# fulcrumgenomics/fgumi

Hardware: AMD Instinct MI355X
Metric: simplex consensus throughput, input raw reads/s (depth-8 x 150bp) (higher is better)
Workload: dtype f64

## Files before the change

### fgumi_amd/csrc/api.cpp

```cpp
#include <chrono>
#include <cstdio>
#include <stdexcept>
#include <cstring>
#include <mutex>
#include <map>
#include <mutex>
#include <string>
#include <thread>
#include "engine.h"
#include <gnu/libc-version.h>
#include <cmath>
#include "fastpath.h"
#include "host_common.h"
#include "simgen.h"
#include "canon_core.h"
#include "reject_core.h"
#include "aln_tags_core.h"

namespace fgx {
using canon::CANON_KIND_DUPLEX; using canon::CANON_KIND_CODEC; using canon::CANON_KIND_SIMPLEX;
uint32_t launch_canon_molecules(hipStream_t s, int kind, const canon::Params& P, const canon::CodecParams& PC, const uint8_t* d_blob,
                                const uint64_t* d_rec_off, const uint32_t* d_rec_len, const uint32_t* d_grp_first, const uint32_t* d_def, uint32_t nd,
                                const uint64_t* d_first, uint8_t* d_out, const uint64_t* d_out_off, uint32_t* d_out_len, int* d_status,
                                canon::Delta* d_delta, DevBuf& slabs, canon::RefRuns* d_runs, const rej::Params* PS);
// ... 1361 lines not shown
  out4[0] = out4[1] = out4[2] = out4[3] = 0;
  if (c && c->fast) { const FastPath& f = c->fast->fp; out4[0] = f.last_packed_families; out4[1] = f.last_classic_families; out4[2] = f.last_split_build; out4[3] = f.last_first_stage_retries; }
}
void fgx_debug_split_first_slice(double mean_records, int packed, uint32_t* out4) {
  if (!out4) return;
  out4[0] = s2_first_slice_bytes(mean_records, packed != 0);
  out4[1] = out4[0] - s2_tile_bytes(mean_records);
  out4[2] = (uint32_t)sizeof(FullItem);
  out4[3] = S2_FLAG_DESC_BYTES;
}
void fgx_debug_last_packed_rows(const fgx_caller* c, uint64_t* out2) {
  if (!out2) return;
  out2[0] = out2[1] = 0;
  if (c && c->fast) { out2[0] = c->fast->fp.last_packed_clean; out2[1] = c->fast->fp.last_packed_general; }
}
void fgx_debug_last_full_results(const fgx_caller* c, uint64_t* out4) {
  if (!out4) return;
  for (int i = 0; i < 4; i++) out4[i] = (c && c->fast) ? c->fast->fp.last_full_results[i] : 0;
}
uint64_t fgx_debug_last_full_results_over(const fgx_caller* c) { return (c && c->fast) ? c->fast->fp.last_full_results[4] : 0; }
int fgx_debug_full_range_whole(uint32_t base, uint32_t items, uint32_t cap) { return full_range_whole(base, items, cap) ? 1 : 0; }
void fgx_debug_last_chain(const fgx_caller* c, uint32_t* out2) { if (out2) { out2[0] = (c && c->fast) ? c->fast->fp.last_launches : 0u; out2[1] = (c && c->fast) ? c->fast->fp.last_host_syncs : 0u; } }
uint32_t fgx_debug_last_routed(const fgx_caller* c) { return (c && c->fast) ? c->fast->fp.last_routed : 0u; }
int fgx_debug_last_direct(const fgx_caller* c) { return (c && c->fast) ? c->fast->fp.last_direct : 0; }
void fgx_set_general_only(fgx_caller* c, int on) { if (c) c->general_only = on != 0; }
void fgx_set_fast_lds_bytes(fgx_caller* c, uint32_t bytes) { if (c) { if (!c->fast) c->fast = new FastState(); c->fast->fp.lds_tile_bytes_large = bytes; } }

int fgx_call_columns(fgx_caller* c, const uint8_t* bases, const uint8_t* quals, uint32_t n_cols, uint32_t depth, uint8_t* out_base,
                     uint8_t* out_qual, uint32_t* out_depth, uint32_t* out_errors) {
  if (!c) return 1;
// ... 143 lines not shown
```

### fgumi_amd/csrc/fastpath.h

```cpp
#pragma once
#include <algorithm>
#include "engine.h"

#if defined(__HIPCC__)
#define FP_HD __host__ __device__ __forceinline__
#else
#define FP_HD inline
#endif

namespace fgx {

constexpr int FAST_RX_CAP = 48;

struct EndDesc {
  uint64_t col_off;
  uint64_t first_off;
  uint64_t kept_off;
  uint32_t cons_len;
  uint32_t rec_size;
  uint16_t mi_off, cb_off;
  uint8_t mi_len, cb_len, rx_len, type;
  uint8_t has_cb, has_rx, valid, meth;
  char rx[FAST_RX_CAP];
};
// ... 41 lines not shown
  return mean_need > floor16 ? std::min<uint32_t>((mean_need + 15u) & ~15u, 17408u) : floor16;
}
constexpr uint32_t FULL_ITEM_OBS = 0x80000000u;
constexpr uint32_t FULL_ITEM_CONT = 0x40000000u;

struct FullResult {
  uint32_t w0;
  uint32_t w1;
};
static_assert(sizeof(FullResult) == 8, "a result is one 8-byte store");
constexpr uint32_t FULL_RESULT_NONE = 0xFFu;
constexpr uint32_t FULL_RESULT_MAX_ITEMS = 64;
#ifndef FGX_FULL_RESULTS_DEFAULT
#define FGX_FULL_RESULTS_DEFAULT 1
#endif
constexpr int FULL_STATS_N = 5, FULL_STATS_STRIDE = 8;
FP_HD uint64_t full_range_word(uint32_t first, uint32_t items, bool whole) {
  return (uint64_t)first | ((uint64_t)(items < 0xFFFFu ? items : 0xFFFFu) << 32) | ((uint64_t)(whole ? 1u : 0u) << 48);
}
FP_HD bool full_range_whole(uint32_t base, uint32_t items, uint32_t cap) { return base < cap && items <= cap - base; }
FP_HD bool emit_pair_takes(uint32_t Lc1, uint32_t Lc2, uint32_t name_len, uint32_t rg_len, uint32_t mi_len, uint32_t cbl1, uint32_t cbl2,
                                                uint32_t rxl1, uint32_t rxl2, bool same_first, uint64_t dcol, uint64_t dout) {
  return Lc1 >= 8u && Lc1 <= 256u && Lc2 >= 8u && Lc2 <= 256u && name_len + 1u <= 32u && rg_len + 4u <= 32u && mi_len + 4u <= 32u &&
         cbl1 + 4u <= 32u && cbl2 + 4u <= 32u && rxl1 + 4u <= 32u && rxl2 + 4u <= 32u && rxl1 <= (uint32_t)FAST_RX_CAP && rxl2 <= (uint32_t)FAST_RX_CAP &&
         same_first && dcol < (1ull << 30) && dout - 1ull < (1ull << 30) - 1ull;
}
FP_HD bool full_results_family(bool packed, bool pair, bool whole, uint32_t items, bool pair_taken) {
  return packed && pair && whole && items <= FULL_RESULT_MAX_ITEMS && pair_taken;
}

struct SplitRec {
// ... 22 lines not shown
  uint16_t qc, sc;
};
struct SplitOut {
  uint8_t status;
  uint8_t ne;
  uint8_t type_a;
  uint8_t fk_a, fk_b;
  uint8_t kept_a, kept_b;
  uint8_t n;
  uint16_t lc_a, lc_b;
  uint32_t rej;
  uint32_t ov_agree, ov_dis, ov_corr;
  uint32_t depth_stats;
};
static_assert(sizeof(SplitRec) == 32 && sizeof(SplitFam) == 32 && sizeof(SplitOut) == 32, "split descriptors are moved as two 16-byte pieces");

struct SlotDesc {
  uint64_t out_off;
  uint32_t lc_seq;
  uint32_t sum_depth;
};
constexpr uint64_t FULL_DEST_DIRECT = 1ull << 62;

struct FastParams {
  const uint8_t* blob; const uint64_t* rec_off; const uint32_t* rec_len; const uint32_t* grp_first;
  uint32_t g0;
  const DeviceTables* T; const DeviceTables* TU;
  uint32_t min_reads; int64_t max_reads;
  char tag0, tag1, cell0, cell1;
  uint32_t min_input_bq, min_cons_bq, trim, overlap, per_base_tags, track_rejects;
// ... 98 lines not shown
  uint32_t last_deep_families = 0;
  DevBuf d_deep_sizes, d_deep_row0, d_deep_rows, d_deep_fams, d_deep_out, d_deep_out2;
  DevBuf d_deep_walk;
  uint32_t last_duplex_deep = 0;
  uint32_t last_duplex_deep_capped = 0;
  bool canon_second_pass = false;
  bool rejects_pass = false;
  uint32_t last_wide_families = 0;
  DevBuf d_wide_scratch, d_wide_pass, d_wide_pass0, d_wide_depth;
  DevBuf d_mflag, d_mu, d_mt, d_mslot, d_mcontigs;
  const void* ref_runs = nullptr;
  uint32_t last_meth_device = 0;
  uint32_t last_meth_clipped = 0;
  uint32_t last_routed = 0;
  uint64_t last_packed_clean = 0, last_packed_general = 0;
  uint64_t last_packed_families = 0, last_classic_families = 0;
  uint32_t last_split_build = 0;
  uint32_t last_first_stage_retries = 0;
  uint32_t last_launches = 0, last_host_syncs = 0;
  DevBuf d_dir_size, d_dir_off, d_dir_base, d_slot_desc, d_slot_err, d_out2, d_scan_tmp2;
  bool direct_off = false;
  uint64_t dir_cap_min = 0;
  uint32_t dir_chunks_run = 0;
  int last_direct = 0;
  uint32_t lds_wave_bytes = 6144;
  uint32_t lds_wave_bytes_duplex = 8704;
  uint32_t lds_wave_bytes_codec = 5120;
  hipEvent_t ev[4] = {nullptr, nullptr, nullptr, nullptr};
  uint32_t pool_slack = 256; bool pool_init = false;
  uint32_t pool_div = 8;
// ... 13 lines not shown
```

### fgumi_amd/csrc/fastpath.hip

```cpp
#if !defined(FGX_WAVEMU)
#include <hipcub/hipcub.hpp>
#endif
#include "bamrec.h"
#include "canon_core.h"
#include "engine.h"
#include <cstdlib>
#include <memory>
#include <string>
#include <type_traits>
#include "fastpath.h"
#include "gate_core.h"
#include "packed_core.h"
#include "record_core.h"

#if defined(FGX_WAVEMU)
#define FGX_DYN_LDS(name) uint8_t* const name = wavemu::dyn_lds()
#define FGX_PIN(...) ((void)0)
#define FGX_UNDEF4(a, b, c, d) do { a = 0; b = 0; c = 0; d = 0; } while (0)
#define FGX_MEM_PIN() ((void)0)
#define FGX_CONST_AS
#else
#define FGX_DYN_LDS(name) extern __shared__ __align__(16) uint8_t name[]
#define FGX_PIN(...) asm volatile("" : __VA_ARGS__)
#define FGX_UNDEF4(a, b, c, d) asm volatile("" : "=v"(a), "=v"(b), "=v"(c), "=v"(d))
// ... 2547 lines not shown
  uint32_t lb = mx > 33 ? (mx - 33) * 2 / 3 + 1 : 1;
  uint32_t ends = (b - a) < max_ends ? (b - a) : max_ends;
  bound[g] = (uint64_t)ends * lb + COL_BOUND_PAD;
  uint64_t lo = 0;
  uint32_t span = 0xFFFFFFFFu;
  if (b > a) {
    lo = rec_off[a];
    const uint64_t hi = rec_off[b - 1] + rec_len[b - 1];
    if (hi >= lo && hi - lo < 0xFFFFFFFFull) span = (uint32_t)(hi - lo);
  }
  fam_desc[g] = make_uint4((uint32_t)lo, (uint32_t)(lo >> 32), span, b - a);
}

__global__ void k_reduce_stats(const unsigned long long* __restrict__ slots, unsigned long long* __restrict__ out, const unsigned long long* __restrict__ full_stats, uint32_t full_out) {
  uint32_t k = threadIdx.x;
  if (k >= 32 && k < 32 + FULL_STATS_N) {
    unsigned long long v = 0;
    for (int i = 0; i < STAT_SLOTS; i++) v += full_stats[(size_t)i * FULL_STATS_STRIDE + (k - 32)];
    out[full_out + (k - 32)] = v;
  }
  if (k >= 32) return;
  unsigned long long v = 0;
  for (int i = 0; i < STAT_SLOTS; i++) v += slots[(size_t)i * 32 + k];
  out[k < FGX_STATS_LEN ? k : 40 + (k - FGX_STATS_LEN)] = v;
}

}

#define FGX_SYNC(st) do { fp.last_host_syncs++; hip_check(hipStreamSynchronize(st), "sync"); } while (0)
#define FGX_LAUNCH(kernel, grid, block, lds, st, ...) do { fp.last_launches++; hipLaunchKernelGGL((kernel), grid, block, lds, st, __VA_ARGS__); hip_check(hipGetLastError(), #kernel " launch"); } while (0)

// ... 16 lines not shown
enum MiscWord : uint32_t {
  MISC_STATS = 0,
  MISC_COLS_USED = 28,
  MISC_N_DEFERRED = 29,
  MISC_N_METH_CLIPPED = 30,
  MISC_N_RETRY = 31,
  MISC_N_RETRY_OLD = 32,
  MISC_N_ROUTE = 33,
  MISC_SMALL_RECS = 35,
  MISC_DIR_FLAGS = 36,
  MISC_N_BIG = 37,
  MISC_N_DEEP = 38,
  MISC_BUILD_FAMILIES = 40,
  MISC_N_SLOW = 44,
  MISC_FULL_RESULTS = 46,
  MISC_READ_BACK = 51,
  MISC_WORDS = 52
};
constexpr uint32_t MISC_SPLIT_WINDOW = MISC_N_BIG - MISC_N_RETRY + 1;
static_assert(FGX_STATS_LEN <= MISC_COLS_USED && MISC_BUILD_FAMILIES == 40 && MISC_BUILD_FAMILIES + (32 - FGX_STATS_LEN) <= MISC_N_SLOW,
              "k_reduce_stats writes words [0, FGX_STATS_LEN) and 40 .. of misc");
static_assert(MISC_N_METH_CLIPPED == MISC_N_DEFERRED + 1 && MISC_N_METH_CLIPPED < MISC_READ_BACK, "meth_clipped_counter: the word behind the deferred count");
static_assert(MISC_N_RETRY < MISC_N_ROUTE && MISC_N_ROUTE < MISC_N_BIG && MISC_SPLIT_WINDOW == 7 && MISC_N_SLOW < MISC_READ_BACK && MISC_READ_BACK <= MISC_WORDS, "misc layout");

inline bool env_not0(const char* e) { return !(e && e[0] == '0'); }
inline bool env_is1(const char* e) { return e && e[0] == '1'; }
inline int env_int(const char* e, int dflt) { return e ? atoi(e) : dflt; }
inline uint32_t env_in(const char* e, int lo, int hi, uint32_t dflt) { const int v = e ? atoi(e) : 0; return v >= lo && v <= hi ? (uint32_t)v : dflt; }

struct ProcessSwitches {
  const bool v2 = env_not0(fgx_knob("FGX_V2")), seg = env_not0(fgx_knob("FGX_SEG"));
  const bool seg2 = env_is1(fgx_knob("FGX_SEG2"));
  const bool early = env_not0(fgx_knob("FGX_S2_EARLY"));
  const int chunks = env_int(getenv("FGX_SPLIT_CHUNKS"), 0);
  const int nosum = env_int(fgx_knob("FGX_S2_NOSUM"), 1);
  const int packed = env_int(getenv("FGX_S2_PACKED"), 1);
  const bool clean_rows = env_not0(getenv("FGX_S2_CLEAN_ROWS"));
  const bool full_results = FGX_FULL_RESULTS_DEFAULT ? env_not0(getenv("FGX_FULL_RESULTS")) : env_is1(getenv("FGX_FULL_RESULTS"));
  const int s2_debug = env_int(fgx_knob("FGX_S2_DEBUG"), 0);
  const int pace = env_int(fgx_knob("FGX_S2_PACE"), 1);
  const uint32_t s2_bytes = env_in(fgx_knob("FGX_S2_BYTES"), 2048, 32768, 0) & ~15u, s2_wpb = env_in(fgx_knob("FGX_S2_WPB"), 1, 4, 0);
  const int s2_partner = env_int(fgx_knob("FGX_S2_PARTNER"), -1);
  const int s2_fixed = env_int(fgx_knob("FGX_S2_FIXED"), -1);
  const bool later_packed = env_not0(fgx_knob("FGX_S2_LATER_PACKED"));
  const bool verbose = env_is1(fgx_knob("FGX_S2_VERBOSE"));
  const uint32_t seg_wpb = env_in(fgx_knob("FGX_SEG_WPB"), 1, WAVES_PER_BLOCK, WAVES_PER_BLOCK), w2_wpb = env_in(fgx_knob("FGX_W2_WPB"), 1, WAVES_PER_BLOCK, FGX_W2_WPB_DEFAULT),
                 fw_wpb = env_in(fgx_knob("FGX_FW_WPB"), 1, WAVES_PER_BLOCK, WAVES_PER_BLOCK);
};
struct BatchSwitches {
  const char* const split_env = getenv("FGX_SPLIT");
  const bool split = env_not0(split_env);
  const int split_mode = env_int(split_env, 1);
// ... 99 lines not shown
    }
    return d.p;
  }
  FastParams stage_params(uint32_t bytes, bool retry) {
    hip_check(hipMemsetAsync(cnt(MISC_N_RETRY), 0, 4, s), "memset");
    FastParams PS = P;
    PS.group_list = cur_list; PS.lds_wave_bytes = bytes;
    PS.retry = retry ? lists[out_list] : nullptr; PS.n_retry = cnt(MISC_N_RETRY);
    return PS;
  }
  void next_list(uint32_t n) { cur_list = lists[out_list]; n_cur = n; out_list ^= 1; }

  void set_up() {
    fp.last_meth_device = 0; fp.last_meth_clipped = 0; fp.last_direct = 0; fp.last_split_chunks = 0;
    if (!fp.canon_second_pass) fp.last_duplex_deep = fp.last_duplex_deep_capped = 0;
    fp.last_routed = 0; fp.last_big_families = 0; fp.last_deep_families = 0; fp.last_wide_families = 0; fp.last_packed_families = 0; fp.last_classic_families = 0; fp.last_packed_clean = 0; fp.last_packed_general = 0; for (uint64_t& v : fp.last_full_results) v = 0; fp.last_split_build = 0; fp.last_first_stage_retries = 0;
    fp.d_ends.reserve((size_t)n_slots * (duplex ? sizeof(DuplexDesc) : codec ? sizeof(CodecDesc) : sizeof(EndDesc)));
    fp.d_sizes.reserve(((size_t)n_slots + 1) * 8);
    fp.d_offsets.reserve(((size_t)n_slots + 1) * 8);
    fp.d_deferred.reserve((size_t)n_grp * 4);
    fp.d_misc.reserve(MISC_WORDS * 8);
    hip_check(hipMemsetAsync(fp.d_misc.p, 0, MISC_WORDS * 8, s), "memset");
    misc = fp.d_misc.as<unsigned long long>();
    const std::string strs = c->prefix + c->rg;
    fp.d_strings.reserve(strs.size() + 16);
    if (!strs.empty()) hip_check(hipMemcpyAsync(fp.d_strings.p, strs.data(), strs.size(), hipMemcpyHostToDevice, s), "H2D strings");
    for (int i = 0; i < 4; i++) if (!fp.ev[i]) hip_check(hipEventCreate(&fp.ev[i]), "hipEventCreate");
    fp.d_bound.reserve(((size_t)n_grp + 1) * 8); fp.d_colbase.reserve(((size_t)n_grp + 1) * 8);
    fp.d_statslots.reserve((size_t)STAT_SLOTS * 32 * 8);
    hip_check(hipMemsetAsync(fp.d_statslots.p, 0, (size_t)STAT_SLOTS * 32 * 8, s), "memset");
    fp.d_famdesc.reserve((size_t)n_grp * 16);
// ... 36 lines not shown
      fp.d_mflag.reserve(col_cap + 64); fp.d_mu.reserve(col_cap * 2 + 64); fp.d_mt.reserve(col_cap * 2 + 64);
      fp.d_mslot.reserve((size_t)n_slots * (meth_dup ? sizeof(DuplexMethSlot) : sizeof(MethSlot)) + 64);
    }
    if (duplex) fp.d_obs.reserve(col_cap * 4); else fp.d_depth.reserve(col_cap * 2 + 64);
    if (dup_cap) fp.d_obs_all.reserve(col_cap * 4);
  }

  void fill_params() {
    memset(&P, 0, sizeof(P));
    P.blob = d_blob; P.rec_off = d_rec_off; P.rec_len = d_rec_len; P.grp_first = d_grp_first;
    P.blob_len = blob_len;
    P.T = c->d_tables.as<DeviceTables>(); P.TU = c->d_umi_tables.as<DeviceTables>();
    P.fw_image = table_image<FwLds>(fp.d_fwimg, build_fw_image, "H2D fw image");
    P.min_reads = o.min_reads; P.max_reads = o.max_reads;
    P.min_input_bq = o.min_input_base_quality; P.min_cons_bq = o.min_consensus_base_quality;
    P.s2_packed = (ps.packed ? 1u : 0u) | ((ps.packed && ps.s2_debug) ? 2u : 0u) | ((ps.packed && ps.clean_rows) ? 4u : 0u);
    P.s2_nsafe = ps.nosum ? unanimous_cap_depth(c->h_tables.t, (uint32_t)o.min_input_base_quality & 0xFFu, 64u) : FGX_NEVER_CAP;
    P.trim = o.trim; P.overlap = o.overlapping_consensus;
    if (duplex) {
      P.min_reads = 1; P.max_reads = -1; P.min_cons_bq = FGX_MIN_PHRED;
      P.dmin_total = o.duplex_min_reads[0]; P.dmin_xy = o.duplex_min_reads[1]; P.dmin_yx = o.duplex_min_reads[2];
      P.dmax_reads = o.duplex_max_reads_per_strand;
      P.col_obs = fp.d_obs.as<uint32_t>(); P.dends = fp.d_ends.as<DuplexDesc>();
      if (dup_cap) P.col_obs_all = fp.d_obs_all.as<uint32_t>();
    }
    if (codec) {
      P.min_reads = 1; P.max_reads = -1; P.min_cons_bq = 0; P.trim = 0; P.overlap = 0;
      P.cends = fp.d_ends.as<CodecDesc>(); P.cmin_reads = o.codec_min_reads_per_strand; P.cmax_reads = o.codec_max_reads_per_strand;
      P.cmin_duplex_len = o.codec_min_duplex_length;
    }
    P.per_base_tags = o.produce_per_base_tags; P.track_rejects = o.track_rejects;
// ... 595 lines not shown
    res->d_out = out_ptr;
    res->out_len = out_len;
    res->count = h_misc[MISC_STATS + 1];
    for (int i = 0; i < FGX_STATS_LEN; i++) res->stats[i] = h_misc[MISC_STATS + i];
    res->n_deferred = (uint32_t)(h_misc[MISC_N_DEFERRED] & 0xFFFFFFFFull);
    fp.last_meth_clipped = (uint32_t)(h_misc[MISC_N_METH_CLIPPED] & 0xFFFFFFFFull);
    if (dup_deep_ran) { fp.last_duplex_deep = (uint32_t)(h_misc[MISC_N_DEEP] & 0xFFFFFFFFull); fp.last_duplex_deep_capped = (uint32_t)(h_misc[MISC_N_DEEP] >> 32); }
    res->d_deferred = fp.d_deferred.as<uint32_t>();
    res->d_out_off = fp.d_offsets.as<uint64_t>();
    res->d_slot_size = fp.d_sizes.as<uint64_t>();
    res->n_slots = n_slots;
    res->ms_kernels = ms; res->ms_k_family = msf; res->ms_k_emit = mse;
    fp.last_packed_families = h_misc[MISC_BUILD_FAMILIES]; fp.last_classic_families = h_misc[MISC_BUILD_FAMILIES + 1];
    fp.last_packed_clean = h_misc[MISC_BUILD_FAMILIES + 2]; fp.last_packed_general = h_misc[MISC_BUILD_FAMILIES + 3];
    for (int i = 0; i < FULL_STATS_N; i++) fp.last_full_results[i] = h_misc[MISC_FULL_RESULTS + i];
    res->cols_used = h_misc[MISC_COLS_USED];
    res->full_items = n_full;
  }
};

int run_once(FastPath& fp, fgx_caller* c, const uint8_t* d_blob, uint64_t blob_len, const uint64_t* d_rec_off, const uint32_t* d_rec_len, uint32_t n_rec,
             const uint32_t* d_grp_first, uint32_t n_grp, FastResult* res) {
  memset(res, 0, sizeof(*res));
  fp.last_launches = 0; fp.last_host_syncs = 0;
  if (n_grp == 0) return 0;
  static const ProcessSwitches ps{};
  Batch b{fp, c, d_blob, blob_len, d_rec_off, d_rec_len, n_rec, d_grp_first, n_grp, res, ps};
  b.set_up();
  b.parse_first_chunk_early();
  b.bound_columns();
// ... 50 lines not shown
```

### fgumi_amd/csrc/packed_core.h

```cpp
#pragma once
#include <cstdint>
#include "consensus_math.h"

namespace fgx {
namespace pk {

constexpr uint32_t H = 0x80808080u;

FGX_HD uint32_t perm(uint32_t a, uint32_t b, uint32_t sel) {
#if defined(__HIP_DEVICE_COMPILE__)
  return __builtin_amdgcn_perm(a, b, sel);
#else
  const unsigned long long src = ((unsigned long long)a << 32) | b;
  uint32_t r = 0;
  for (int i = 0; i < 4; i++) {
    const uint32_t s = (sel >> (8 * i)) & 0xFFu;
    const uint32_t byte = s < 8u ? (uint32_t)(src >> (8 * s)) & 0xFFu : 0u;
    r |= byte << (8 * i);
  }
  return r;
#endif
}
FGX_HD uint32_t bitrev32(uint32_t x) {
#if defined(__HIP_DEVICE_COMPILE__)
// ... 85 lines not shown
    const uint32_t Vh = h ? (uint32_t)(V >> 32) : (uint32_t)V;
    const uint32_t Z = O & ((O | H) - 0x01010101u) & 0x0F0F0F0Fu;
    const uint32_t nzO = (O + 0x7F7F7F7Fu) & H, nzZ = (Z + 0x7F7F7F7Fu) & H;
    const uint32_t ge = ((C | H) - N4) & H;
    const uint32_t capF = Vh & nzO & ~nzZ & ge;
    o.flag2[h] = Vh & nzO & ~capF;
    o.valid2[h] = Vh;
    const uint32_t capM = (capF << 1) - (capF >> 7);
    o.code2[h] = cap_lt ? 0x0F0F0F0Fu : ((O & capM) | (0x0F0F0F0Fu & ~capM));
    o.qual2[h] = (QA4 & capM) | (QZ4 & ~capM);
    const uint32_t D = C & capM;
    o.dep4[2 * h] = perm(0u, D, 0x0C010C00u); o.dep4[2 * h + 1] = perm(0u, D, 0x0C030C02u);
  }
}

inline void fill_t1(uint8_t* t1 , const ConsensusTables& t) {
  for (uint32_t q = 0; q < 96; q++) {
    t1[q] = 0xFF;
    if (q > 93) continue;
    ColumnAcc acc;
    acc.reset();
    acc.add(0, t.correct[q], t.error_per_alt[q]);
    if (!m_isfinite(acc.s[0]) || !m_isfinite(acc.s[1])) continue;
    int bi = -1;
    uint8_t ql = 0;
    column_call(t, acc.s, acc.obs, &bi, &ql);
    if (bi == 0) t1[q] = ql;
  }
}

// ... 21 lines not shown
```

### fgumi_amd/csrc/simplex_split.inc

```

#ifndef FGX_S2_OCC
#define FGX_S2_OCC 6
#endif
#ifndef FGX_S2_OCC_PACKED
#define FGX_S2_OCC_PACKED 7
#endif
#ifndef FGX_S2_PAIRS
#define FGX_S2_PAIRS 256
#endif

#ifndef FGX_S2_F32
#define FGX_S2_F32 1
#endif
#ifndef FGX_S2_FMASEL
#define FGX_S2_FMASEL 1
#endif
#ifndef FGX_S2_NOSUM
#define FGX_S2_NOSUM 1
#endif
#ifndef FGX_S2_PREGATE
#define FGX_S2_PREGATE 1
#endif
struct S2Lds {
  GateTables g;
// ... 676 lines not shown
      const uint32_t x1 = drop ? c1 : agree ? 0u : (c1 ^ cb), x2 = drop ? c2 : agree ? 0u : (c2 ^ cb);
      const bool changed = nq != qa || nq != qb;
      if (valid) {
        atomicXor((uint32_t*)(W + (o1 & ~3u)), x1 << (8 * (o1 & 3) + sh1));
        atomicXor((uint32_t*)(W + (o2 & ~3u)), x2 << (8 * (o2 & 3) + sh2));
        W[q1] = (uint8_t)newq; W[q2] = (uint8_t)newq;
      }
      const uint32_t na = (uint32_t)__popcll(__ballot(valid && agree)), nd = (uint32_t)__popcll(__ballot(valid && !agree));
      ov_agree += na; ov_dis += nd;
      ov_corr += (uint32_t)__popcll(__ballot(valid && agree && changed)) + 2u * nd;
    };
    const unsigned long long om = __ballot(act && ov_cnt != 0);
    if (om) {
      const uint32_t np = (uint32_t)__popcll(om), fp = (uint32_t)__builtin_ctzll(om);
      const uint32_t cn0 = rlane(ov_cnt, fp);
      if (ov_uniform && np > 1u && cn0 < 64u) {
        const uint32_t oo1 = rlane(ov_off1, fp), oo2 = rlane(ov_off2, fp);
        if (act && ov_cnt != 0) *(uint16_t*)(W + ibase + 2u * (uint32_t)__popcll(om & below)) = (uint16_t)(slot | (mate_slot << 8));
        wave_sync();
        const uint32_t inv = uni((uint32_t)(1048576.0f / (float)cn0) + 2u);
        const uint32_t total = np * cn0;
        for (uint32_t t0 = 0; t0 < total; t0 += 64) {
          const uint32_t t = t0 + lane;
          const bool in = t < total;
          const uint32_t tt = in ? t : 0u;
          const uint32_t pk = s2_mul24(tt, inv) >> 20, w = tt - s2_mul24(pk, cn0);
          const uint32_t rows = *(const uint16_t*)(W + ibase + 2u * pk), r1 = rows & 0xFF, r2 = rows >> 8;
          const uint32_t i1 = oo1 + w, i2 = oo2 + w;
          shared_base(in, S0 + r1 * SS + (i1 >> 1), S0 + r2 * SS + (i2 >> 1), r1 * QS + i1, r2 * QS + i2, (~i1 & 1) << 2, (~i2 & 1) << 2);
        }
      } else {
        const uint32_t mt_q = mate_slot * QS, mt_s = S0 + mate_slot * SS;
        const uint32_t my_q0 = slot * QS, my_s0 = S0 + slot * SS;
        for (unsigned long long pm = om; pm; pm &= pm - 1) {
          const uint32_t a = (uint32_t)__builtin_ctzll(pm);
          const uint32_t sa = rlane(my_s0, a), qa0 = rlane(my_q0, a), sb = rlane(mt_s, a), qb0 = rlane(mt_q, a);
          const uint32_t cn = rlane(ov_cnt, a);
          const uint32_t i1 = rlane(ov_off1, a) + lane, i2 = rlane(ov_off2, a) + lane;
          uint32_t o1 = sa + (i1 >> 1), o2 = sb + (i2 >> 1), q1 = qa0 + i1, q2 = qb0 + i2;
          const uint32_t sh1 = (~i1 & 1) << 2, sh2 = (~i2 & 1) << 2;
          for (uint32_t w0 = 0; w0 < cn; w0 += 64, o1 += 32, o2 += 32, q1 += 64, q2 += 64) shared_base(w0 + lane < cn, o1, o2, q1, q2, sh1, sh2);
        }
      }
    }
  }
  const uint32_t ov_bases = ov_agree + ov_dis;
  wave_sync();
  PH(3)
  S2_ABLATE_AFTER(3, ov_bases + ov_corr + W[my_s])

  const uint32_t fl = l_seq > clip ? l_seq - clip : 0u;
  if (act) {
    uint32_t z0, z1;
    if (!rev) { z0 = fl; z1 = ty == 2u ? len_b : len_a; } else { z0 = 0; z1 = clip < l_seq ? clip : l_seq; }
    if (z0 < z1) {
      if (z0 & 1u) { W[my_s + (z0 >> 1)] &= 0xF0; z0++; }
      if (z0 < z1 && (z1 & 1u)) { W[my_s + (z1 >> 1)] &= 0x0F; z1--; }
      for (uint32_t b = z0 >> 1; b < (z1 >> 1); b++) W[my_s + b] = 0;
// ... 630 lines not shown
    else if (threadIdx.x == 24u) tiny_w = w[(offsetof(S2Lds, g) + offsetof(GateTables, cap)) / 4];
  } else {
#pragma unroll
    for (int u = 0; u < 6; u++) { const uint32_t ii = threadIdx.x + u * blockDim.x; im[u] = img_src[ii < IMG_V ? ii : 0u]; }
  }
  uint8_t* W = dyn + (size_t)wv * P.lds_wave_bytes;
  const uint32_t my_list = blockIdx.x & (N_LISTS - 1);
  s2_cols_family<QS_T, SS_T, DIRECT, COLS, false>(P, g, bail, tiny_w, im, W, sL, lane, my_list);
}

__global__ __launch_bounds__(256) void k_split_finish(FastParams P, uint32_t count) {
  typedef uint32_t u32x4 __attribute__((ext_vector_type(4)));
  const uint32_t gi = blockIdx.x * blockDim.x + threadIdx.x;
  const uint32_t lane = threadIdx.x & 63;
  uint32_t c_total = 0, c_cons = 0, c_insuf = 0, c_zero = 0, c_orphan = 0, c_agree = 0, c_dis = 0, c_corr = 0, c_packed = 0, c_classic = 0, c_clean = 0;
  uint32_t c_apply = 0, c_cut = 0, c_over = 0;
  if (gi < count) {
    const uint32_t g = P.group_list ? P.group_list[gi] : P.g0 + gi;
    const SplitOut O = P.split_out[g];
    const uint32_t slot0 = 3 * g;
    const uint32_t o_status = O.status & 0x3Fu;
    const bool padded = (O.status & 0x80u) != 0;
    const bool clean = (O.status & 0x40u) != 0;
    if (o_status == 2) { c_total = O.n; c_insuf = O.n; }
    const bool direct = P.out != nullptr;
    if (o_status != 0 && !direct) {
      EndDesc* D = &P.ends[slot0];
      D[0].valid = 0; D[1].valid = 0; D[2].valid = 0;
      P.rec_sizes[slot0] = 0; P.rec_sizes[slot0 + 1] = 0; P.rec_sizes[slot0 + 2] = 0;
    }
    if (o_status == 1) {
      c_packed = padded ? 1u : 0u; c_classic = padded ? 0u : 1u; c_clean = (padded && clean) ? 1u : 0u;
      c_total = O.n; c_cons = O.ne;
      c_insuf = O.rej & 0xFF; c_zero = (O.rej >> 8) & 0xFF; c_orphan = O.rej >> 16;
      c_agree = O.ov_agree; c_dis = O.ov_dis; c_corr = O.ov_corr;
      const uint4 fd = P.fam_desc[g];
      const unsigned long long lo_off = (unsigned long long)fd.x | ((unsigned long long)fd.y << 32);
      const uint32_t r0 = P.grp_first[g];
      const SplitFam F = P.split_fam[g];
      const SplitRec R0 = P.split_rec[r0];
      const uint64_t col_base = P.col_base[g];
      if (direct) {
        const uint8_t* const fbase = P.blob + lo_off;
        const uint8_t* const strs = (const uint8_t*)P.strings;
        const uint32_t mi0 = R0.mi_len, nm = P.prefix_len + 1u + mi0;
        const uint8_t* const mi_src = fbase + R0.mi_rel;
        uint64_t rec_off = P.dir_off[g];
        for (uint32_t k = 0; k < O.ne; k++) {
          const uint32_t Lc = k == 0 ? O.lc_a : O.lc_b, e_type = k == 0 ? O.type_a : 2u;
          const uint32_t fk = k == 0 ? O.fk_a : O.fk_b, kept = k == 0 ? O.kept_a : O.kept_b;
// ... 95 lines not shown
      }
      if (fr_pair) {
        const uint32_t items = (uint32_t)(fr_word >> 32) & 0xFFFFu;
        const bool whole = ((fr_word >> 48) & 1u) != 0;
        const bool taken = emit_pair_takes(O.lc_a, O.lc_b, P.prefix_len + 1u + R0.mi_len, P.rg_len, R0.mi_len, fr_cbl[0], fr_cbl[1], fr_rxl[0], fr_rxl[1], true,
                                           (uint64_t)(s2_padded_b(O.lc_a) - S2_PAD_FRONT), (uint64_t)fr_size0 + 4ull);
        if (full_results_family(true, true, whole, items, taken)) { c_apply = 1u; P.full_flag[g] = 1; }
        else if (taken) { if (!whole) c_cut = 1u; else c_over = 1u; }
      }
    }
  }
  const uint32_t t_cons = wave_sum(c_cons), t_total = wave_sum(c_total), t_insuf = wave_sum(c_insuf), t_zero = wave_sum(c_zero), t_orphan = wave_sum(c_orphan);
  const uint32_t t_agree = wave_sum(c_agree), t_dis = wave_sum(c_dis), t_corr = wave_sum(c_corr);
  const uint32_t t_packed = wave_sum(c_packed), t_classic = wave_sum(c_classic);
  const uint32_t t_clean = wave_sum(c_clean);
  if (lane == 0) {
    unsigned long long* st = P.stats + (size_t)((blockIdx.x * 4 + (threadIdx.x >> 6)) & (STAT_SLOTS - 1)) * 32;
    if (t_total) atomicAdd(&st[0], (unsigned long long)t_total);
    if (t_cons) atomicAdd(&st[1], (unsigned long long)t_cons);
    const uint32_t filt = t_insuf + t_zero + t_orphan;
    if (filt) atomicAdd(&st[2], (unsigned long long)filt);
    if (t_insuf) atomicAdd(&st[3 + FGX_REJ_INSUFFICIENT_READS], (unsigned long long)t_insuf);
    if (t_zero) atomicAdd(&st[3 + FGX_REJ_ZERO_LENGTH_AFTER_TRIMMING], (unsigned long long)t_zero);
    if (t_orphan) atomicAdd(&st[3 + FGX_REJ_ORPHAN_CONSENSUS], (unsigned long long)t_orphan);
    if (t_agree + t_dis) atomicAdd(&st[24], (unsigned long long)(t_agree + t_dis));
    if (t_agree) atomicAdd(&st[25], (unsigned long long)t_agree);
    if (t_dis) atomicAdd(&st[26], (unsigned long long)t_dis);
    if (t_corr) atomicAdd(&st[27], (unsigned long long)t_corr);
    if (t_packed) atomicAdd(&st[28], (unsigned long long)t_packed);
    if (t_classic) atomicAdd(&st[29], (unsigned long long)t_classic);
    if (t_clean) atomicAdd(&st[30], (unsigned long long)t_clean);
    if (t_packed - t_clean) atomicAdd(&st[31], (unsigned long long)(t_packed - t_clean));
  }
  if (P.full_results) {
    const uint32_t t_apply = wave_sum(c_apply), t_cut = wave_sum(c_cut), t_over = wave_sum(c_over);
    if (lane == 0) {
      unsigned long long* fs = P.full_stats + (size_t)((blockIdx.x * 4 + (threadIdx.x >> 6)) & (STAT_SLOTS - 1)) * FULL_STATS_STRIDE;
      if (t_apply) atomicAdd(&fs[2], (unsigned long long)t_apply);
      if (t_cut) atomicAdd(&fs[3], (unsigned long long)t_cut);
      if (t_over) atomicAdd(&fs[4], (unsigned long long)t_over);
    }
  }
}
```

Before: 3.161 billion.

## Process overlapping mate pairs in packed SWAR form within split consensus kernel

Adds a packed overlap-consensus path that works on 8 bases per lane using byte-wise SWAR arithmetic on packed quality and nibble base words, instead of the per-base bytewise overlap loop. Mate bytes are gathered with alignbyte/alignbit and updates are scattered back with atomic XORs. A guard pass falls back to the bytewise path when high-bit qualities appear. The path is on by default for single-column packed families. It adds overlap-path counters to the stats reduction, and the XOR scatter and guard pre-pass add complexity and extra work.

```diff
diff --git a/fgumi_amd/csrc/api.cpp b/fgumi_amd/csrc/api.cpp
--- a/fgumi_amd/csrc/api.cpp
+++ b/fgumi_amd/csrc/api.cpp
@@ -1399,6 +1399,10 @@
   out2[0] = out2[1] = 0;
   if (c && c->fast) { out2[0] = c->fast->fp.last_packed_clean; out2[1] = c->fast->fp.last_packed_general; }
 }
+void fgx_debug_last_packed_overlap(const fgx_caller* c, uint64_t* out3) {
+  if (!out3) return;
+  for (int i = 0; i < 3; i++) out3[i] = (c && c->fast) ? c->fast->fp.last_packed_overlap[i] : 0;
+}
 void fgx_debug_last_full_results(const fgx_caller* c, uint64_t* out4) {
   if (!out4) return;
   for (int i = 0; i < 4; i++) out4[i] = (c && c->fast) ? c->fast->fp.last_full_results[i] : 0;
diff --git a/fgumi_amd/csrc/fastpath.h b/fgumi_amd/csrc/fastpath.h
--- a/fgumi_amd/csrc/fastpath.h
+++ b/fgumi_amd/csrc/fastpath.h
@@ -79,7 +79,8 @@
 #ifndef FGX_FULL_RESULTS_DEFAULT
 #define FGX_FULL_RESULTS_DEFAULT 1
 #endif
-constexpr int FULL_STATS_N = 5, FULL_STATS_STRIDE = 8;
+constexpr int FULL_STATS_N = 5, FULL_STATS_STRIDE = 8, OV_STATS_N = 3;
+static_assert(FULL_STATS_N + OV_STATS_N <= FULL_STATS_STRIDE, "the overlap counters share the slots of the result counters");
 FP_HD uint64_t full_range_word(uint32_t first, uint32_t items, bool whole) {
   return (uint64_t)first | ((uint64_t)(items < 0xFFFFu ? items : 0xFFFFu) << 32) | ((uint64_t)(whole ? 1u : 0u) << 48);
 }
@@ -132,6 +133,7 @@
   uint32_t depth_stats;
 };
 static_assert(sizeof(SplitRec) == 32 && sizeof(SplitFam) == 32 && sizeof(SplitOut) == 32, "split descriptors are moved as two 16-byte pieces");
+constexpr uint32_t S2_OV_COUNT = 0x0FFFFFFFu, S2_OV_PACKED = 1u << 28, S2_OV_BYTEWISE = 1u << 29, S2_OV_GUARD = 1u << 30;
 
 struct SlotDesc {
   uint64_t out_off;
@@ -260,6 +262,7 @@
   uint32_t last_meth_clipped = 0;
   uint32_t last_routed = 0;
   uint64_t last_packed_clean = 0, last_packed_general = 0;
+  uint64_t last_packed_overlap[OV_STATS_N] = {0, 0, 0};
   uint64_t last_packed_families = 0, last_classic_families = 0;
   uint32_t last_split_build = 0;
   uint32_t last_first_stage_retries = 0;
diff --git a/fgumi_amd/csrc/fastpath.hip b/fgumi_amd/csrc/fastpath.hip
--- a/fgumi_amd/csrc/fastpath.hip
+++ b/fgumi_amd/csrc/fastpath.hip
@@ -2585,7 +2585,7 @@
 
 __global__ void k_reduce_stats(const unsigned long long* __restrict__ slots, unsigned long long* __restrict__ out, const unsigned long long* __restrict__ full_stats, uint32_t full_out) {
   uint32_t k = threadIdx.x;
-  if (k >= 32 && k < 32 + FULL_STATS_N) {
+  if (k >= 32 && k < 32 + FULL_STATS_N + OV_STATS_N) {
     unsigned long long v = 0;
     for (int i = 0; i < STAT_SLOTS; i++) v += full_stats[(size_t)i * FULL_STATS_STRIDE + (k - 32)];
     out[full_out + (k - 32)] = v;
@@ -2632,13 +2632,15 @@
   MISC_BUILD_FAMILIES = 40,
   MISC_N_SLOW = 44,
   MISC_FULL_RESULTS = 46,
-  MISC_READ_BACK = 51,
-  MISC_WORDS = 52
+  MISC_PACKED_OVERLAP = 51,
+  MISC_READ_BACK = 54,
+  MISC_WORDS = 56
 };
 constexpr uint32_t MISC_SPLIT_WINDOW = MISC_N_BIG - MISC_N_RETRY + 1;
 static_assert(FGX_STATS_LEN <= MISC_COLS_USED && MISC_BUILD_FAMILIES == 40 && MISC_BUILD_FAMILIES + (32 - FGX_STATS_LEN) <= MISC_N_SLOW,
               "k_reduce_stats writes words [0, FGX_STATS_LEN) and 40 .. of misc");
 static_assert(MISC_N_METH_CLIPPED == MISC_N_DEFERRED + 1 && MISC_N_METH_CLIPPED < MISC_READ_BACK, "meth_clipped_counter: the word behind the deferred count");
+static_assert(MISC_PACKED_OVERLAP == MISC_FULL_RESULTS + FULL_STATS_N && MISC_PACKED_OVERLAP + OV_STATS_N <= MISC_READ_BACK, "k_reduce_stats writes the overlap counters behind the result counters");
 static_assert(MISC_N_RETRY < MISC_N_ROUTE && MISC_N_ROUTE < MISC_N_BIG && MISC_SPLIT_WINDOW == 7 && MISC_N_SLOW < MISC_READ_BACK && MISC_READ_BACK <= MISC_WORDS, "misc layout");
 
 inline bool env_not0(const char* e) { return !(e && e[0] == '0'); }
@@ -2654,6 +2656,7 @@
   const int nosum = env_int(fgx_knob("FGX_S2_NOSUM"), 1);
   const int packed = env_int(getenv("FGX_S2_PACKED"), 1);
   const bool clean_rows = env_not0(getenv("FGX_S2_CLEAN_ROWS"));
+  const bool packed_overlap = env_not0(getenv("FGX_S2_PACKED_OVERLAP"));
   const bool full_results = FGX_FULL_RESULTS_DEFAULT ? env_not0(getenv("FGX_FULL_RESULTS")) : env_is1(getenv("FGX_FULL_RESULTS"));
   const int s2_debug = env_int(fgx_knob("FGX_S2_DEBUG"), 0);
   const int pace = env_int(fgx_knob("FGX_S2_PACE"), 1);
@@ -2783,7 +2786,7 @@
   void set_up() {
     fp.last_meth_device = 0; fp.last_meth_clipped = 0; fp.last_direct = 0; fp.last_split_chunks = 0;
     if (!fp.canon_second_pass) fp.last_duplex_deep = fp.last_duplex_deep_capped = 0;
-    fp.last_routed = 0; fp.last_big_families = 0; fp.last_deep_families = 0; fp.last_wide_families = 0; fp.last_packed_families = 0; fp.last_classic_families = 0; fp.last_packed_clean = 0; fp.last_packed_general = 0; for (uint64_t& v : fp.last_full_results) v = 0; fp.last_split_build = 0; fp.last_first_stage_retries = 0;
+    fp.last_routed = 0; fp.last_big_families = 0; fp.last_deep_families = 0; fp.last_wide_families = 0; fp.last_packed_families = 0; fp.last_classic_families = 0; fp.last_packed_clean = 0; fp.last_packed_general = 0; for (uint64_t& v : fp.last_packed_overlap) v = 0; for (uint64_t& v : fp.last_full_results) v = 0; fp.last_split_build = 0; fp.last_first_stage_retries = 0;
     fp.d_ends.reserve((size_t)n_slots * (duplex ? sizeof(DuplexDesc) : codec ? sizeof(CodecDesc) : sizeof(EndDesc)));
     fp.d_sizes.reserve(((size_t)n_slots + 1) * 8);
     fp.d_offsets.reserve(((size_t)n_slots + 1) * 8);
@@ -2850,7 +2853,7 @@
     P.fw_image = table_image<FwLds>(fp.d_fwimg, build_fw_image, "H2D fw image");
     P.min_reads = o.min_reads; P.max_reads = o.max_reads;
     P.min_input_bq = o.min_input_base_quality; P.min_cons_bq = o.min_consensus_base_quality;
-    P.s2_packed = (ps.packed ? 1u : 0u) | ((ps.packed && ps.s2_debug) ? 2u : 0u) | ((ps.packed && ps.clean_rows) ? 4u : 0u);
+    P.s2_packed = (ps.packed ? 1u : 0u) | ((ps.packed && ps.s2_debug) ? 2u : 0u) | ((ps.packed && ps.clean_rows) ? 4u : 0u) | ((ps.packed && ps.packed_overlap) ? 8u : 0u);
     P.s2_nsafe = ps.nosum ? unanimous_cap_depth(c->h_tables.t, (uint32_t)o.min_input_base_quality & 0xFFu, 64u) : FGX_NEVER_CAP;
     P.trim = o.trim; P.overlap = o.overlapping_consensus;
     if (duplex) {
@@ -3476,6 +3479,7 @@
     fp.last_packed_families = h_misc[MISC_BUILD_FAMILIES]; fp.last_classic_families = h_misc[MISC_BUILD_FAMILIES + 1];
     fp.last_packed_clean = h_misc[MISC_BUILD_FAMILIES + 2]; fp.last_packed_general = h_misc[MISC_BUILD_FAMILIES + 3];
     for (int i = 0; i < FULL_STATS_N; i++) fp.last_full_results[i] = h_misc[MISC_FULL_RESULTS + i];
+    for (int i = 0; i < OV_STATS_N; i++) fp.last_packed_overlap[i] = h_misc[MISC_PACKED_OVERLAP + i];
     res->cols_used = h_misc[MISC_COLS_USED];
     res->full_items = n_full;
   }
diff --git a/fgumi_amd/csrc/packed_core.h b/fgumi_amd/csrc/packed_core.h
--- a/fgumi_amd/csrc/packed_core.h
+++ b/fgumi_amd/csrc/packed_core.h
@@ -123,6 +123,98 @@
   }
 }
 
+FGX_HD uint32_t alignbyte(uint32_t hi, uint32_t lo, uint32_t n) {
+#if defined(__HIP_DEVICE_COMPILE__)
+  return __builtin_amdgcn_alignbyte(hi, lo, n);
+#else
+  return (uint32_t)(((((unsigned long long)hi) << 32) | lo) >> (8u * (n & 3u)));
+#endif
+}
+FGX_HD uint32_t alignbit(uint32_t hi, uint32_t lo, uint32_t n) {
+#if defined(__HIP_DEVICE_COMPILE__)
+  return __builtin_amdgcn_alignbit(hi, lo, n);
+#else
+  return (uint32_t)(((((unsigned long long)hi) << 32) | lo) >> (n & 31u));
+#endif
+}
+FGX_HD uint32_t popc(uint32_t x) {
+#if defined(__HIP_DEVICE_COMPILE__)
+  return (uint32_t)__builtin_popcount(x);
+#else
+  x = x - ((x >> 1) & 0x55555555u); x = (x & 0x33333333u) + ((x >> 2) & 0x33333333u);
+  return (((x + (x >> 4)) & 0x0F0F0F0Fu) * 0x01010101u) >> 24;
+#endif
+}
+FGX_HD uint32_t widen(uint32_t h) { return h - (h >> 7); }
+FGX_HD uint32_t swap_nibbles(uint32_t x) { return ((x & 0x0F0F0F0Fu) << 4) | ((x >> 4) & 0x0F0F0F0Fu); }
+FGX_HD uint32_t expand_bam(uint32_t c, int h) { const uint32_t P = perm(c, c, h ? 0x03030202u : 0x01010000u); return ((P >> 4) & 0x000F000Fu) | (P & 0x0F000F00u); }
+FGX_HD uint32_t expand_pos(uint32_t c, int h) { const uint32_t P = perm(c, c, h ? 0x03030202u : 0x01010000u); return (P & 0x000F000Fu) | ((P >> 4) & 0x0F000F00u); }
+FGX_HD uint32_t compress_bam(uint32_t lo, uint32_t hi) { return perm((hi << 4) | (hi >> 8), (lo << 4) | (lo >> 8), 0x06040200u); }
+FGX_HD uint32_t compress_pos(uint32_t lo, uint32_t hi) { return perm(hi | (hi >> 4), lo | (lo >> 4), 0x06040200u); }
+
+FGX_HD void ov_in_masks(uint32_t cn, uint32_t k, uint32_t* ml, uint32_t* mh) {
+  const uint32_t nv = cn > 8u * k ? cn - 8u * k : 0u;
+  const unsigned long long m = nv >= 8u ? ~0ull : (1ull << (8u * nv)) - 1ull;
+  *ml = (uint32_t)m; *mh = (uint32_t)(m >> 32);
+}
+FGX_HD void ov_gather_q(uint32_t d0, uint32_t d1, uint32_t d2, uint32_t s, uint32_t* qx, uint32_t* qy) { *qx = alignbyte(d1, d0, s); *qy = alignbyte(d2, d1, s); }
+FGX_HD uint32_t ov_gather_c(uint32_t w0, uint32_t w1, uint32_t sn) { return alignbit(swap_nibbles(w1), swap_nibbles(w0), 4u * sn); }
+FGX_HD void ov_scatter_q(uint32_t dx, uint32_t dy, uint32_t s, uint32_t* e ) {
+  const unsigned long long D = (((unsigned long long)dy) << 32) | dx, L = D << (8u * s);
+  e[0] = (uint32_t)L; e[1] = (uint32_t)(L >> 32); e[2] = (uint32_t)((D >> 8) >> (56u - 8u * s));
+}
+FGX_HD void ov_scatter_c(uint32_t d, uint32_t sn, uint32_t* f ) {
+  f[0] = swap_nibbles(d << (4u * sn)); f[1] = swap_nibbles((d >> 4) >> (28u - 4u * sn));
+}
+FGX_HD bool ov_high(uint32_t qax, uint32_t qay, uint32_t qbx, uint32_t qby, uint32_t ml, uint32_t mh) { return ((((qax | qbx) & ml) | ((qay | qby) & mh)) & H) != 0u; }
+
+struct OvHalf { uint32_t newq, newc, validM, agree, dis, chg; };
+FGX_HD void ov_half(uint32_t qa, uint32_t qb, uint32_t ca, uint32_t cb, uint32_t inr, uint32_t mb4, OvHalf& o) {
+  const uint32_t L = 0x7F7F7F7Fu;
+  qa &= L; qb &= L;
+  const uint32_t isN = ((ca + 0x71717171u) | (cb + 0x71717171u)) & H;
+  const uint32_t ne = ((ca ^ cb) + L) & H;
+  const uint32_t valid = inr & ~isN & H;
+  const uint32_t s = qa + qb;
+  const uint32_t overM = widen((s | ((s & L) + 0x22222222u)) & H);
+  const uint32_t nq = ((s & L) & ~overM) | (0x5D5D5D5Du & overM);
+  const uint32_t xg = (qa | H) - qb, yg = (qb | H) - qa;
+  const uint32_t ageM = widen(xg & H);
+  const uint32_t ad = ((xg & ageM) | (yg & ~ageM)) & L;
+  const uint32_t lt2M = widen(~((ad | H) - 0x02020202u) & H);
+  const uint32_t dq = (ad & ~lt2M) | (0x02020202u & lt2M);
+  const uint32_t neM = widen(ne);
+  o.newq = (dq & neM) | (nq & ~neM);
+  const uint32_t dropM = widen(~((o.newq | H) - mb4) & H);
+  o.newc = (((ca & ageM) | (cb & ~ageM)) | (0x0F0F0F0Fu & widen(xg & yg & ne))) & ~dropM;
+  o.validM = widen(valid);
+  o.agree = valid & ~ne; o.dis = valid & ne;
+  o.chg = o.agree & (((nq ^ qa) | (nq ^ qb)) + L);
+}
+#if defined(__HIP_DEVICE_COMPILE__)
+#define FGX_PK_THEN(a, b, c, d, e, f, g, h, i, j) asm volatile("" : "+v"(a), "+v"(b), "+v"(c), "+v"(d), "+v"(e), "+v"(f), "+v"(g), "+v"(h), "+v"(i), "+v"(j))
+#else
+#define FGX_PK_THEN(a, b, c, d, e, f, g, h, i, j) ((void)0)
+#endif
+struct OvStep { uint32_t qa[2], ca, dq[2], dc, n_ad, n_chg; };
+FGX_HD void ov_step(uint32_t qax, uint32_t qay, uint32_t caw, uint32_t qbx, uint32_t qby, uint32_t cbp, uint32_t ml, uint32_t mh, uint32_t mb4, OvStep& o) {
+  uint32_t a8[2], d8[2];
+  o.n_ad = 0; o.n_chg = 0;
+#pragma unroll
+  for (int h = 0; h < 2; h++) {
+    const uint32_t qa = h ? qay : qax, qb = h ? qby : qbx, ca = expand_bam(caw, h), cb = expand_pos(cbp, h);
+    OvHalf r;
+    ov_half(qa, qb, ca, cb, h ? mh : ml, mb4, r);
+    o.qa[h] = (r.newq & r.validM) | (qa & ~r.validM);
+    a8[h] = (r.newc & r.validM) | (ca & ~r.validM);
+    o.dq[h] = (r.newq ^ qb) & r.validM;
+    d8[h] = (r.newc ^ cb) & r.validM;
+    o.n_ad += popc(r.agree) + (popc(r.dis) << 16); o.n_chg += popc(r.chg);
+    if (h == 0) FGX_PK_THEN(o.qa[0], a8[0], o.dq[0], d8[0], o.n_ad, o.n_chg, qay, qby, caw, cbp);
+  }
+  o.ca = compress_bam(a8[0], a8[1]); o.dc = compress_pos(d8[0], d8[1]);
+}
+
 inline void fill_t1(uint8_t* t1 , const ConsensusTables& t) {
   for (uint32_t q = 0; q < 96; q++) {
     t1[q] = 0xFF;
diff --git a/fgumi_amd/csrc/simplex_split.inc b/fgumi_amd/csrc/simplex_split.inc
--- a/fgumi_amd/csrc/simplex_split.inc
+++ b/fgumi_amd/csrc/simplex_split.inc
@@ -714,7 +714,65 @@
     if (om) {
       const uint32_t np = (uint32_t)__popcll(om), fp = (uint32_t)__builtin_ctzll(om);
       const uint32_t cn0 = rlane(ov_cnt, fp);
-      if (ov_uniform && np > 1u && cn0 < 64u) {
+      bool ov_packed = false, ov_guard = false;
+      if constexpr (COLS == 1) {
+        const uint32_t oo1 = rlane(ov_off1, fp), oo2 = rlane(ov_off2, fp);
+        if ((KA::of(P).s2_packed & 8u) && ov_uniform && np > 1u && (oo1 == 0u || oo2 == 0u) && ((QS & 7u) | (SS & 3u)) == 0u && min_bq <= 128u) {
+          if (act && ov_cnt != 0) *(uint16_t*)(W + ibase + 2u * (uint32_t)__popcll(om & below)) = (uint16_t)(slot | (mate_slot << 8));
+          wave_sync();
+          const bool a_is_1 = oo1 == 0u;
+          const uint32_t off = oo1 | oo2, sq = off & 3u, sn = off & 7u;
+          const uint32_t ng = (cn0 + 7u) >> 3, total = np * ng;
+          const uint32_t inv = uni((uint32_t)(1048576.0f / (float)ng) + 2u);
+          const uint32_t mb4 = min_bq * 0x01010101u;
+          struct OvLane { uint32_t aq, as, bq, bs, ml, mh, qax, qay, caw, qbx, qby, cbp; };
+          auto ov_load = [&](const uint32_t t0, OvLane& L) {
+            const uint32_t t = t0 + lane;
+            const bool in = t < total;
+            const uint32_t tt = in ? t : 0u;
+            const uint32_t pi = s2_mul24(tt, inv) >> 20, k = tt - s2_mul24(pi, ng);
+            const uint32_t rows = *(const uint16_t*)(W + ibase + 2u * pi), r1 = rows & 0xFF, r2 = rows >> 8;
+            const uint32_t rA = a_is_1 ? r1 : r2, rB = a_is_1 ? r2 : r1;
+            L.aq = rA * QS + 8u * k; L.as = S0 + rA * SS + 4u * k;
+            L.bq = rB * QS + 4u * ((off >> 2) + 2u * k); L.bs = S0 + rB * SS + 4u * ((off >> 3) + k);
+            pk::ov_in_masks(in ? cn0 : 0u, k, &L.ml, &L.mh);
+            const uint2 qa = *(const uint2*)(W + L.aq);
+            L.qax = qa.x; L.qay = qa.y; L.caw = *(const uint32_t*)(W + L.as);
+            pk::ov_gather_q(*(const uint32_t*)(W + L.bq), *(const uint32_t*)(W + L.bq + 4u), *(const uint32_t*)(W + L.bq + 8u), sq, &L.qbx, &L.qby);
+            L.cbp = pk::ov_gather_c(*(const uint32_t*)(W + L.bs), *(const uint32_t*)(W + L.bs + 4u), sn);
+          };
+          if (total > 64u) {
+            uint32_t hi_v = 0;
+            for (uint32_t t0 = 0; t0 < total; t0 += 64) { OvLane L; ov_load(t0, L); hi_v |= pk::ov_high(L.qax, L.qay, L.qbx, L.qby, L.ml, L.mh) ? 1u : 0u; }
+            ov_guard = __any(hi_v != 0u);
+          }
+          if (!ov_guard) {
+            uint32_t n_ad = 0, n_chg = 0;
+            for (uint32_t t0 = 0; t0 < total; t0 += 64) {
+              OvLane L;
+              ov_load(t0, L);
+              if (total <= 64u && __any(pk::ov_high(L.qax, L.qay, L.qbx, L.qby, L.ml, L.mh))) { ov_guard = true; break; }
+              pk::OvStep R;
+              pk::ov_step(L.qax, L.qay, L.caw, L.qbx, L.qby, L.cbp, L.ml, L.mh, mb4, R);
+              uint32_t e[3], f[2];
+              pk::ov_scatter_q(R.dq[0], R.dq[1], sq, e); pk::ov_scatter_c(R.dc, sn, f);
+              if (t0 + lane < total) {
+                *(uint2*)(W + L.aq) = make_uint2(R.qa[0], R.qa[1]); *(uint32_t*)(W + L.as) = R.ca;
+                atomicXor((uint32_t*)(W + L.bq), e[0]); atomicXor((uint32_t*)(W + L.bq + 4u), e[1]); atomicXor((uint32_t*)(W + L.bq + 8u), e[2]);
+                atomicXor((uint32_t*)(W + L.bs), f[0]); atomicXor((uint32_t*)(W + L.bs + 4u), f[1]);
+              }
+              n_ad += R.n_ad; n_chg += R.n_chg;
+            }
+            if (!ov_guard) {
+              const uint32_t t_ad = wave_sum(n_ad), t_chg = wave_sum(n_chg);
+              ov_agree = t_ad & 0xFFFFu; ov_dis = t_ad >> 16; ov_corr = t_chg + 2u * ov_dis;
+              ov_packed = true;
+            }
+          }
+        }
+      }
+      if (ov_packed) {
+      } else if (ov_uniform && np > 1u && cn0 < 64u) {
         const uint32_t oo1 = rlane(ov_off1, fp), oo2 = rlane(ov_off2, fp);
         if (act && ov_cnt != 0) *(uint16_t*)(W + ibase + 2u * (uint32_t)__popcll(om & below)) = (uint16_t)(slot | (mate_slot << 8));
         wave_sync();
@@ -742,6 +800,7 @@
           for (uint32_t w0 = 0; w0 < cn; w0 += 64, o1 += 32, o2 += 32, q1 += 64, q2 += 64) shared_base(w0 + lane < cn, o1, o2, q1, q2, sh1, sh2);
         }
       }
+      if constexpr (COLS == 1) ov_corr |= ov_packed ? S2_OV_PACKED : ov_guard ? (S2_OV_BYTEWISE | S2_OV_GUARD) : S2_OV_BYTEWISE;
     }
   }
   const uint32_t ov_bases = ov_agree + ov_dis;
@@ -1402,6 +1461,7 @@
   const uint32_t gi = blockIdx.x * blockDim.x + threadIdx.x;
   const uint32_t lane = threadIdx.x & 63;
   uint32_t c_total = 0, c_cons = 0, c_insuf = 0, c_zero = 0, c_orphan = 0, c_agree = 0, c_dis = 0, c_corr = 0, c_packed = 0, c_classic = 0, c_clean = 0;
+  uint32_t c_ovp = 0, c_ovb = 0, c_ovg = 0;
   uint32_t c_apply = 0, c_cut = 0, c_over = 0;
   if (gi < count) {
     const uint32_t g = P.group_list ? P.group_list[gi] : P.g0 + gi;
@@ -1421,7 +1481,8 @@
       c_packed = padded ? 1u : 0u; c_classic = padded ? 0u : 1u; c_clean = (padded && clean) ? 1u : 0u;
       c_total = O.n; c_cons = O.ne;
       c_insuf = O.rej & 0xFF; c_zero = (O.rej >> 8) & 0xFF; c_orphan = O.rej >> 16;
-      c_agree = O.ov_agree; c_dis = O.ov_dis; c_corr = O.ov_corr;
+      c_agree = O.ov_agree; c_dis = O.ov_dis; c_corr = O.ov_corr & S2_OV_COUNT;
+      if (padded) { c_ovp = (O.ov_corr & S2_OV_PACKED) ? 1u : 0u; c_ovb = (O.ov_corr & S2_OV_BYTEWISE) ? 1u : 0u; c_ovg = (O.ov_corr & S2_OV_GUARD) ? 1u : 0u; }
       const uint4 fd = P.fam_desc[g];
       const unsigned long long lo_off = (unsigned long long)fd.x | ((unsigned long long)fd.y << 32);
       const uint32_t r0 = P.grp_first[g];
@@ -1547,6 +1608,7 @@
   const uint32_t t_agree = wave_sum(c_agree), t_dis = wave_sum(c_dis), t_corr = wave_sum(c_corr);
   const uint32_t t_packed = wave_sum(c_packed), t_classic = wave_sum(c_classic);
   const uint32_t t_clean = wave_sum(c_clean);
+  const uint32_t t_ovp = wave_sum(c_ovp), t_ovb = wave_sum(c_ovb), t_ovg = wave_sum(c_ovg);
   if (lane == 0) {
     unsigned long long* st = P.stats + (size_t)((blockIdx.x * 4 + (threadIdx.x >> 6)) & (STAT_SLOTS - 1)) * 32;
     if (t_total) atomicAdd(&st[0], (unsigned long long)t_total);
@@ -1564,6 +1626,12 @@
     if (t_classic) atomicAdd(&st[29], (unsigned long long)t_classic);
     if (t_clean) atomicAdd(&st[30], (unsigned long long)t_clean);
     if (t_packed - t_clean) atomicAdd(&st[31], (unsigned long long)(t_packed - t_clean));
+    if (t_ovp | t_ovb) {
+      unsigned long long* fs = P.full_stats + (size_t)((blockIdx.x * 4 + (threadIdx.x >> 6)) & (STAT_SLOTS - 1)) * FULL_STATS_STRIDE + FULL_STATS_N;
+      if (t_ovp) atomicAdd(&fs[0], (unsigned long long)t_ovp);
+      if (t_ovb) atomicAdd(&fs[1], (unsigned long long)t_ovb);
+      if (t_ovg) atomicAdd(&fs[2], (unsigned long long)t_ovg);
+    }
   }
   if (P.full_results) {
     const uint32_t t_apply = wave_sum(c_apply), t_cut = wave_sum(c_cut), t_over = wave_sum(c_over);
```

Result: faster. 3.262 billion, median of 6 (+3.2%).
